# GinZhu/RDST

Measured on AMD Instinct MI355X. Metric: SR patches/sec fwd+bwd, RDST-E1 x4 64->256, higher is better.
Workload: dtype bf16; 1 GPU; RDST-E1 x4 (RDST_E1_OASIS_example_SRx4.ini), 1x64x64 LR patches -> 256x256, step = fwd + L1 + bwd + flat-bucket grad all-reduce + Adam; global_batch=32, per_gpu_batch=32, parallelism=dp1, hip_graph=True, grad_bucket_bytes=17859844

## Files before the change

### include/rdst_hip.h

```cpp
#ifndef RDST_HIP_H
#define RDST_HIP_H

#include <stddef.h>
#include <stdint.h>

#ifdef __cplusplus
extern "C" {
#endif

#define RDST_F32 0
#define RDST_BF16 1
#define RDST_F32X3 2

#define RDST_EINVAL (-10001)
#define RDST_ENOTSUP (-10002)

#define RDST_ACT_NONE 0
#define RDST_ACT_GELU 1
#define RDST_ACT_LEAKY02 2
#define RDST_ACT_LEAKY001 3

int rdst_abi_version(void);
const char* rdst_last_error(void);

// ... 81 lines not shown

#define RDST_PREPACKED ((size_t)-1)
#define RDST_PACK_LINEAR 0
#define RDST_PACK_CONV3_FWD 1
#define RDST_PACK_LINEAR_SEC3 2
#define RDST_PACK_LINEAR_X3 3
#define RDST_PACK_CONV3_FWD_X3 4
typedef struct rdst_pack_job {
  int kind;
  const float* W; const float* gamma; const float* beta; const float* bias;
  void* out;
  int N, K;
  float s;
} rdst_pack_job;
int rdst_pack_batch(const rdst_pack_job* jobs, int njobs, void* stream);
int rdst_ln_linear_fwd_packable(int K, int N, int has_ln, int has_residual, int in_act, int dtype);
size_t rdst_conv_fwd_workspace2(int Cin, int Cout, int ksize, int dtype);
int rdst_conv_fwd_packable(int Cin, int Cout, int ksize, int shuffle_r, int has_residual, int in_act, int dtype);

int rdst_reduce_batch_begin(void);
int rdst_reduce_batch_end(void* stream);
int rdst_reduce_batch_abort(void);

int rdst_nchw_to_rows(const float* nchw, void* rows, int64_t ld, int B, int C, int H, int W,
                      int dtype, void* stream);
int rdst_rows_to_nchw(const void* rows, int64_t ld, float* nchw, int B, int C, int H, int W,
                      int dtype, void* stream);

int rdst_upsample2_fwd(const void* x, int64_t ld_x, void* y, int64_t ld_y, int B, int H, int W, int C, int dtype,
                       void* stream);
int rdst_upsample2_bwd(const void* dy, int64_t ld_dy, void* dx, int64_t ld_dx, int B, int H, int W, int C, int dtype,
                       void* stream);

int rdst_adam_step(float* param, const float* grad, float* exp_avg, float* exp_avg_sq, int64_t n,
                   float lr, float beta1, float beta2, float eps, float weight_decay, int64_t step,
                   void* stream);

size_t rdst_u_scratch_bytes(void);

int rdst_u_conv(const void* X1, int64_t ld1, int C1, int up1, const void* X2, int64_t ld2, int C2, const void* Wp,
                const float* bias, const void* add, int64_t ld_add, void* Y, int64_t ld_y, int B, int Hin, int Win, int Hout,
                int Wout, int Cout, int Npad, int ksize, int stride, int transposed, int dtype, void* stream,
                const float* bn1, float* stats, int* stats_blocks);

int rdst_u_stem_fwd(const float* img, const float* W, void* Y, int64_t ld_y, int B, int Cin, int H, int Wd, int dtype,
                    void* stream);
// ... 80 lines not shown
```

### rdst_amd/_lib.py

```python
from __future__ import annotations

import ctypes as C
import os

_HERE = os.path.dirname(os.path.abspath(__file__))
LIB_PATH = os.environ.get("RDST_HIP_LIB") or os.path.join(_HERE, "librdst_hip.so")

F32, BF16, F32X3 = 0, 1, 2
EINVAL, ENOTSUP = -10001, -10002
ACT_NONE, ACT_GELU, ACT_LEAKY02, ACT_LEAKY001 = 0, 1, 2, 3

_p, _i, _l, _f, _z = C.c_void_p, C.c_int, C.c_int64, C.c_float, C.c_size_t


class LrSchedule(C.Structure):
    MAX_MILESTONES = 16
    _fields_ = [("milestones", C.c_int64 * 16), ("lr", C.c_float * 17), ("count", C.c_int32)]


STEP_STATE_BYTES = 48
SKIP_LOSS, SKIP_NONFINITE, SKIP_PEER = 1, 2, 4

SIGNATURES = {
    "rdst_abi_version": (_i, []),
# ... 14 lines not shown
    "rdst_mlp_fwd_packable": (_i, [_i, _i, _i]),
    "rdst_mlp_fwd": (_i, [_p, _l, _p, _p, _p, _p, _p, _p, _p, _l, _p, _p, _z, _l, _i, _i, _i, _p]),
    "rdst_mlp_bwd_workspace": (_z, [_l, _i, _i]),
    "rdst_mlp_bwd": (_i, [_p, _l, _p, _p, _p, _p, _p, _p, _p, _l, _p, _l, _p, _p, _p, _p, _p, _p, _p, _z, _l, _i, _i, _i,
                          _p]),
    "rdst_wattn_fwd_lse": (_i, [_p, _l, _p, _p, _l, _p, _i, _i, _i, _i, _i, _i, _i, _f, _i, _p]),
    "rdst_wattn_bwd_lse": (_i, [_p, _l, _p, _p, _l, _p, _l, _p, _p, _l, _p, _p, _z, _i, _i, _i, _i, _i, _i, _i, _f, _i, _p]),
    "rdst_swin_attn_fwd_supported": (_i, [_i, _i, _i, _i]),
    "rdst_swin_attn_fwd_workspace": (_z, [_i]),
    "rdst_swin_attn_fwd": (_i, [_p, _l, _p, _p, _p, _p, _p, _p, _p, _p, _l, _p, _l, _p, _l, _p, _p, _z, _i, _i, _i, _i, _i, _i, _i,
                                _f, _i, _p]),
    "rdst_conv_fwd_workspace": (_z, [_i, _i, _i]),
    "rdst_conv_fwd_workspace2": (_z, [_i, _i, _i, _i]),
    "rdst_conv_fwd": (_i, [_p, _l, _i, _p, _p, _p, _l, _p, _l, _p, _z, _i, _i, _i, _i, _i, _i, _f, _i, _i, _p]),
    "rdst_conv_bwd_workspace": (_z, [_i, _i, _i, _i, _i, _i]),
    "rdst_conv_bwd": (_i, [_p, _l, _i, _p, _p, _l, _p, _l, _p, _l, _p, _p, _p, _z, _i, _i, _i, _i, _i, _i,
                           _f, _i, _i, _p]),
    "rdst_pack_batch": (_i, [_p, _i, _p]),
    "rdst_ln_linear_fwd_packable": (_i, [_i, _i, _i, _i, _i, _i]),
    "rdst_conv_fwd_packable": (_i, [_i, _i, _i, _i, _i, _i, _i]),
    "rdst_reduce_batch_begin": (_i, []),
    "rdst_reduce_batch_end": (_i, [_p]),
    "rdst_reduce_batch_abort": (_i, []),
    "rdst_wattn_fwd_drop": (_i, [_p, _l, _p, _p, _i, _p, _l, _i, _i, _i, _i, _i, _i, _i, _f, _i, _f, _p, _p]),
    "rdst_wattn_bwd_drop": (_i, [_p, _l, _p, _p, _i, _p, _l, _p, _l, _p, _p, _z, _i, _i, _i, _i, _i, _i, _i, _f, _i, _f, _p, _p]),
    "rdst_wattn_drop_mask": (_i, [_p, _i, _i, _i, _i, _i, _f, _p, _p]),
    "rdst_nchw_to_rows": (_i, [_p, _p, _l, _i, _i, _i, _i, _i, _p]),
    "rdst_rows_to_nchw": (_i, [_p, _l, _p, _i, _i, _i, _i, _i, _p]),
    "rdst_upsample2_fwd": (_i, [_p, _l, _p, _l, _i, _i, _i, _i, _i, _p]),
    "rdst_upsample2_bwd": (_i, [_p, _l, _p, _l, _i, _i, _i, _i, _i, _p]),
    "rdst_adam_step": (_i, [_p, _p, _p, _p, _l, _f, _f, _f, _f, _f, _l, _p]),
    "rdst_u_scratch_bytes": (_z, []),
    "rdst_u_conv": (_i, [_p, _l, _i, _i, _p, _l, _i, _p, _p, _p, _l, _p, _l, _i, _i, _i, _i, _i, _i, _i, _i, _i, _i, _i, _p, _p, _p,
                         C.POINTER(C.c_int)]),
    "rdst_u_bn_stats_from": (_i, [_p, _i, _l, _i, _p, _p, _f, _f, _p, _p, _p, _p, _p]),
    "rdst_u_stem_fwd": (_i, [_p, _p, _p, _l, _i, _i, _i, _i, _i, _p]),
    "rdst_u_stem_dgrad": (_i, [_p, _l, _p, _p, _p, _i, _i, _i, _i, _i, _p]),
    "rdst_u_bn_stats": (_i, [_p, _l, _l, _i, _p, _p, _f, _f, _p, _p, _p, _p, _i, _p]),
    "rdst_u_bn_apply": (_i, [_p, _l, _p, _p, _l, _p, _p, _l, _i, _p, _l, _l, _i, _i, _p]),
    "rdst_u_bn_bwd": (_i, [_p, _l, _p, _l, _p, _l, _p, _p, _l, _p, _l, _p, _l, _l, _i, _p, _i, _p]),
    "rdst_u_maxpool_fwd": (_i, [_p, _l, _p, _l, _p, _i, _i, _i, _i, _i, _p]),
    "rdst_u_maxpool_bwd": (_i, [_p, _l, _p, _p, _l, _p, _l, _i, _i, _i, _i, _i, _p]),
    "rdst_u_sumpool2": (_i, [_p, _l, _p, _l, _p, _l, _i, _i, _i, _i, _i, _p]),
    "rdst_u_pair_loss_fwd": (_i, [_p, _l, _p, _l, _l, _i, _i, _f, _i, _p, _p, _i, _p]),
    "rdst_u_pair_loss_bwd": (_i, [_p, _l, _p, _l, _l, _i, _i, _f, _p, _p, _l, _p, _l, _i, _p]),
    "rdst_u_dice_fwd": (_i, [_p, _l, _p, _l, _p, _l, _i, _i, _f, _f, _i, _p, _p, _p, _i, _p]),
# ... 66 lines not shown
```

### rdst_amd/csrc/conv.h

```cpp
#pragma once
#include "common.h"

struct ConvGeom {
  int B, H, W;
  int Cin, Cout;
  int ks, pad;
  int r;
  __host__ __device__ __forceinline__ int64_t pixels() const { return (int64_t)B * H * W; }
  __device__ __forceinline__ void decode(int64_t p, int& b, int& y, int& x) const {
    const int hw = H * W;
    b = (int)(p / hw);
    const int q = (int)(p - (int64_t)b * hw);
    y = q / W;
    x = q - y * W;
  }
  __device__ __forceinline__ void out_rc(int b, int y, int x, int co, int64_t& row, int& c) const {
    if (r == 1) {
      row = ((int64_t)b * H + y) * W + x;
      c = co;
      return;
    }
    const int r2 = r * r;
    c = co / r2;
    const int rem = co - c * r2, i = rem / r, j = rem - i * r;
    row = ((int64_t)b * (H * r) + y * r + i) * (int64_t)(W * r) + x * r + j;
  }
};

template <typename T>
int conv_fwd_mfma(const T* X, int64_t ldx, int in_act, const float* Wc, const float* bias, const T* R, int64_t ldr,
                  T* Y, int64_t ldy, const ConvGeom& g, float s, bool split, hipStream_t st);
template <typename T>
const T* plain_dy(const T* dY, int64_t lddy, const ConvGeom& g, void* scratch, int64_t& ld_out, hipStream_t st, int& rc);
template <typename T>
int conv_dgrad_mfma(const T* X, int64_t ldx, int in_act, const float* Wc, const T* dYp, int64_t lddyp, T* dX,
                    int64_t lddx, const T* acc, int64_t ldacc, const ConvGeom& g, float s, bool split, hipStream_t st);
template <typename T>
int conv_wgrad_mfma(const T* X, int64_t ldx, int in_act, const T* dYp, int64_t lddyp, float* dW, float* dbias,
                    float* slab, const ConvGeom& g, float s, bool split, hipStream_t st);
size_t conv_mfma_scratch_bytes(const ConvGeom& g);

int conv_c1_fwd_bf16(const bf16* X, int64_t ldx, int in_act, const float* Wc, const float* bias, const bf16* R, int64_t ldr, bf16* Y,
                     int64_t ldy, const ConvGeom& g, float s, hipStream_t st);
int conv_c1_bwd_bf16(const bf16* X, int64_t ldx, int in_act, const float* Wc, const bf16* dY, int64_t lddy, bf16* dX,
                     int64_t lddx, const bf16* acc, int64_t ldacc, float* dW, float* dbias, float* slab, const ConvGeom& g,
                     float s, hipStream_t st);
size_t conv_c1_slab_floats(int Cin);
int conv_in1_fwd_bf16(const bf16* X, int64_t ldx, int in_act, const float* Wc, const float* bias, const bf16* R, int64_t ldr, bf16* Y,
                      int64_t ldy, const ConvGeom& g, float s, hipStream_t st);
int conv_in1_wgrad_bf16(const bf16* X, int64_t ldx, int in_act, const bf16* dY, int64_t lddy, float* dW, float* dbias, float* slab,
                        const ConvGeom& g, float s, hipStream_t st);
size_t conv_in1_slab_floats(int Cout);

size_t conv3_pack_bytes(int Cin, int Cout);
int conv3_fwd_shape(int Cin, int Cout, int ks, int r, bool has_res, int in_act);
int conv3_fwd_bf16(const bf16* X, int64_t ldx, int in_act, const float* Wc, const float* bias, const bf16* R, int64_t ldr,
                   bf16* Y, int64_t ldy, const ConvGeom& g, float s, void* wpack, bool prepacked, hipStream_t st);
int conv3_dgrad_bf16(const float* Wc, const bf16* dY, int64_t lddy, bf16* dX, int64_t lddx, const bf16* acc, int64_t ldacc,
                     int in_act, const ConvGeom& g, float s, void* wpack, hipStream_t st);
size_t conv3_wgrad_slab_bytes(int Cin, int Cout);
int conv3_wgrad_bf16(const bf16* X, int64_t ldx, int in_act, const bf16* dY, int64_t lddy, float* dW, float* dbias, float* slab,
                     const ConvGeom& g, float s, hipStream_t st);

size_t conv3x_pack_bytes(int Cin, int Cout);
int conv3x_fwd_shape(int Cin, int Cout, int ks, int r, bool has_res, int in_act);
int conv3x_fwd_f32(const float* X, int64_t ldx, int in_act, const float* Wc, const float* bias, const float* R, int64_t ldr,
                   float* Y, int64_t ldy, const ConvGeom& g, float s, void* wpack, bool prepacked, hipStream_t st);
int conv3x_dgrad_f32(const float* Wc, const float* dY, int64_t lddy, float* dX, int64_t lddx, const float* acc, int64_t ldacc,
                     int in_act, const ConvGeom& g, float s, void* wpack, hipStream_t st);
// ... 12 lines not shown
```

### rdst_amd/csrc/conv.hip

```cpp
#include "common.h"
#include "gemm_valu.h"
#include "conv.h"

namespace {

template <typename T>
struct ConvA {
  static constexpr bool kFast = true;
  const T* X; int64_t ldx; ConvGeom g; int act;
  __device__ __forceinline__ float operator()(int64_t p, int64_t k) const {
    const int tap = (int)(k / g.Cin), ci = (int)(k - (int64_t)tap * g.Cin);
    const int ky = tap / g.ks, kx = tap - ky * g.ks;
    int b, y, x;
    g.decode(p, b, y, x);
    const int yy = y + ky - g.pad, xx = x + kx - g.pad;
    if (yy < 0 || yy >= g.H || xx < 0 || xx >= g.W) return 0.f;
    return apply_act(to_f32<T>(X[(((int64_t)b * g.H + yy) * g.W + xx) * ldx + ci]), act);
  }
};
template <typename T>
struct ConvAT {
  static constexpr bool kFast = false;
  ConvA<T> a;
  __device__ __forceinline__ float operator()(int64_t p, int n) const { return a(p, n); }
};
// ... 99 lines not shown
int fwd_t(const T* X, int64_t ldx, int in_act, const float* Wc, const float* bias, const T* R, int64_t ldr, T* Y,
          int64_t ldy, const ConvGeom& g, float s, void* wpack, bool prepacked, bool split, hipStream_t st) {
  if constexpr (sizeof(T) == 2) {
    if (int rc = conv_c1_fwd_bf16(X, ldx, in_act, Wc, bias, R, ldr, Y, ldy, g, s, st); rc != RDST_ENOTSUP) return rc;
    if (int rc = conv_in1_fwd_bf16(X, ldx, in_act, Wc, bias, R, ldr, Y, ldy, g, s, st); rc != RDST_ENOTSUP) return rc;
    if (int rc = conv3_fwd_bf16(X, ldx, in_act, Wc, bias, R, ldr, Y, ldy, g, s, wpack, prepacked, st); rc != RDST_ENOTSUP) return rc;
  }
  if constexpr (sizeof(T) == 4) {
    if (int rc = conv_c1x_fwd_f32(X, ldx, in_act, Wc, bias, R, ldr, Y, ldy, g, s, st); rc != RDST_ENOTSUP) return rc;
    if (int rc = conv_in1x_fwd_f32(X, ldx, in_act, Wc, bias, R, ldr, Y, ldy, g, s, st); rc != RDST_ENOTSUP) return rc;
  }
  if constexpr (sizeof(T) == 4) {
    if (split)
      if (int rc = conv3x_fwd_f32(X, ldx, in_act, Wc, bias, R, ldr, Y, ldy, g, s, wpack, prepacked, st); rc != RDST_ENOTSUP) return rc;
  }
  if (int rc = conv_fwd_mfma<T>(X, ldx, in_act, Wc, bias, R, ldr, Y, ldy, g, s, split, st); rc != RDST_ENOTSUP) return rc;
  ConvA<T> la{X, ldx, g, in_act};
  ConvB lb{Wc, g};
  ConvFwdEp<T> ep{bias, R, ldr, Y, ldy, g, s};
  return gemm_valu_launch(la, lb, ep, g.pixels(), g.Cout, (int64_t)g.ks * g.ks * g.Cin, 1, st, "conv_fwd");
}

template <typename T>
int bwd_t(const T* X, int64_t ldx, int in_act, const float* Wc, const T* dY, int64_t lddy, T* dX, int64_t lddx,
          const T* acc, int64_t ldacc, float* dW, float* dbias, float* wsp, const ConvGeom& g, float s, bool split, hipStream_t st) {
  const int64_t wtotal = (int64_t)g.Cout * g.Cin * g.ks * g.ks;
  void* wpack = wsp;
  wsp = reinterpret_cast<float*>(reinterpret_cast<char*>(wsp) + conv3x_pack_bytes(g.Cin, g.Cout));
  float* w3slab = wsp;
  wsp = reinterpret_cast<float*>(reinterpret_cast<char*>(wsp) + (g.ks == 3 ? conv3_wgrad_slab_bytes(g.Cin, g.Cout) : 0));
  float* slab = wsp;
  float* small = slab + (int64_t)kMaxSplits * wtotal;
  char* mscr = reinterpret_cast<char*>(small + (int64_t)kSmallBlocks * g.Cout + 64);
  if constexpr (sizeof(T) == 2) {
    float* c1slab = reinterpret_cast<float*>(mscr + conv_mfma_scratch_bytes(ConvGeom{g.B, g.H, g.W, g.Cin, g.Cout, g.ks, g.pad, 2}));
    if (int rc = conv_c1_bwd_bf16(X, ldx, in_act, Wc, dY, lddy, dX, lddx, acc, ldacc, dW, dbias, c1slab, g, s, st); rc != RDST_ENOTSUP)
      return rc;
    if (!dX && (dW || dbias) && g.r == 1) {
      if (int rc = conv_in1_wgrad_bf16(X, ldx, in_act, dY, lddy, dW, dbias, c1slab, g, s, st); rc != RDST_ENOTSUP) return rc;
    }
  }
  if constexpr (sizeof(T) == 4) {
    float* c1slab = reinterpret_cast<float*>(mscr + conv_mfma_scratch_bytes(ConvGeom{g.B, g.H, g.W, g.Cin, g.Cout, g.ks, g.pad, 2}));
    if (int rc = conv_c1x_bwd_f32(X, ldx, in_act, Wc, dY, lddy, dX, lddx, acc, ldacc, dW, dbias, c1slab, g, s, st); rc != RDST_ENOTSUP)
      return rc;
    if (!dX && (dW || dbias) && g.r == 1) {
      if (int rc = conv_in1x_wgrad_f32(X, ldx, in_act, dY, lddy, dW, dbias, c1slab, g, s, st); rc != RDST_ENOTSUP) return rc;
    }
  }
  bool dxdone = false;
  if constexpr (sizeof(T) == 2) {
    if (dX) {
      const int rc = conv3_dgrad_bf16(Wc, dY, lddy, dX, lddx, acc, ldacc, in_act, g, s, wpack, st);
      if (rc == 0) dxdone = true;
      else if (rc != RDST_ENOTSUP) return rc;
    }
    if (dW || dbias) {
      const int rc = conv3_wgrad_bf16(X, ldx, in_act, dY, lddy, dW, dbias, w3slab, g, s, st);
      if (rc == 0) { dW = nullptr; dbias = nullptr; }
      else if (rc != RDST_ENOTSUP) return rc;
    }
    if ((dxdone || !dX) && !dW && !dbias) return 0;
  }
  if constexpr (sizeof(T) == 4) {
    if (dX && split) {
      const int rc = conv3x_dgrad_f32(Wc, dY, lddy, dX, lddx, acc, ldacc, in_act, g, s, wpack, st);
      if (rc == 0) dxdone = true;
      else if (rc != RDST_ENOTSUP) return rc;
    }
    if ((dW || dbias) && split) {
      const int rc = conv3x_wgrad_f32(X, ldx, in_act, dY, lddy, dW, dbias, w3slab, g, s, st);
      if (rc == 0) { dW = nullptr; dbias = nullptr; }
      else if (rc != RDST_ENOTSUP) return rc;
    }
    if ((dxdone || !dX) && !dW && !dbias) return 0;
  }
  int prc = 0;
  int64_t ldp = lddy;
  const T* dYp = plain_dy<T>(dY, lddy, g, mscr, ldp, st, prc);
  if (prc) return prc;
  float* mslab = reinterpret_cast<float*>(mscr + (g.r > 1 ? (size_t)g.pixels() * g.Cout * 4 : 0));
  bool wdone = false;
  if (dW || dbias) {
    const int rc = conv_wgrad_mfma<T>(X, ldx, in_act, dYp, ldp, dW, dbias, mslab, g, s, split, st);
    if (rc == 0) wdone = true;
    else if (rc != RDST_ENOTSUP) return rc;
  }
  if (!wdone && dbias) {
    ConvDyCol<T> f{dY, lddy, g, s};
    if (int rc = colsum_launch(f, g.pixels(), g.Cout, small, kSmallBlocks, dbias, st, "conv_dbias")) return rc;
  }
  if (!wdone && dW) {
    ConvDyAT<T> la{dY, lddy, g, s};
    ConvAT<T> lb{ConvA<T>{X, ldx, g, in_act}};
    ConvSlabEp ep{slab, g};
    const int splits = wgrad_splits(g);
    const int z = gemm_valu_splits(g.pixels(), splits);
    int rc = gemm_valu_launch(la, lb, ep, g.Cout, g.ks * g.ks * g.Cin, g.pixels(), splits, st, "conv_wgrad");
    if (!rc) rc = slab_reduce(slab, dW, z, wtotal, st);
    if (rc) return rc;
  }
  if (dX && !dxdone) {
    int rc = conv_dgrad_mfma<T>(X, ldx, in_act, Wc, dYp, ldp, dX, lddx, acc, ldacc, g, s, split, st);
    if (rc == RDST_ENOTSUP) {
      ConvDyA<T> la{dY, lddy, g, s};
      ConvBd lb{Wc, g};
      ConvDxEp<T> ep{X, ldx, dX, lddx, in_act, acc, ldacc};
      rc = gemm_valu_launch(la, lb, ep, g.pixels(), g.Cin, (int64_t)g.ks * g.ks * g.Cout, 1, st, "conv_dgrad");
    }
    if (rc) return rc;
  }
  return 0;
}

int make_geom(ConvGeom& g, int B, int H, int W, int Cin, int Cout, int ks, int r, const char* who) {
  if (B <= 0 || H <= 0 || W <= 0 || Cin <= 0 || Cout <= 0) return rdst_fail(RDST_EINVAL, "%s: non-positive dimension", who);
  if (ks != 1 && ks != 3) return rdst_fail(RDST_ENOTSUP, "%s: kernel size %d (1 or 3)", who, ks);
  if (r < 1 || Cout % (r * r)) return rdst_fail(RDST_EINVAL, "%s: Cout=%d not divisible by shuffle^2=%d", who, Cout, r * r);
  if ((int64_t)B * H * W * r * r >= (1ll << 31)) return rdst_fail(RDST_EINVAL, "%s: more than 2^31 output pixels", who);
  g.B = B; g.H = H; g.W = W; g.Cin = Cin; g.Cout = Cout; g.ks = ks; g.pad = ks / 2; g.r = r;
  return 0;
}

template <typename T>
__global__ void __launch_bounds__(256) nchw_to_rows_kernel(const float* __restrict__ src, T* __restrict__ rows, int64_t ld,
                                                           int B, int C, int64_t HW) {
  const int64_t i = (int64_t)blockIdx.x * 256 + threadIdx.x;
  if (i >= (int64_t)B * HW * C) return;
  const int c = (int)(i % C);
  const int64_t bp = i / C, b = bp / HW, p = bp - b * HW;
  rows[bp * ld + c] = from_f32<T>(src[(b * C + c) * HW + p]);
}
template <typename T>
__global__ void __launch_bounds__(256) rows_to_nchw_kernel(const T* __restrict__ rows, int64_t ld, float* __restrict__ dst,
                                                           int B, int C, int64_t HW) {
// ... 95 lines not shown
```

### rdst_amd/csrc/conv_c1.hip

```cpp
#include "common.h"
#include "gemm_valu.h"
#include "conv.h"
#include "mfma.h"

namespace {

typedef float f32x2 __attribute__((ext_vector_type(2)));

struct C1Args {
  const bf16* X; int64_t ldx;
  const float* W;
  const float* bias;
  const bf16* dY; int64_t lddy;
  bf16* Y; int64_t ldy;
  bf16* dX; int64_t lddx; const bf16* Acc; int64_t ldacc;
  float* slab;
  ConvGeom g; float s;
  int tiles_x, tiles_y; int64_t ntiles;
};

constexpr int C1_THREADS = 256;
constexpr int C1_TH = 8, C1_TW = 32, C1_HH = C1_TH + 2, C1_HW = C1_TW + 2, C1_NPIX = C1_HH * C1_HW, C1_PS = 144;

__device__ __forceinline__ void c1_unpack8(const u32x4_a4& v, float (&f)[8]) {
// ... 423 lines not shown
  hipLaunchKernelGGL(conv_c1_dgrad_kernel<true>, dim3(grid), dim3(C1_THREADS), 0, st, p);
  return rdst_launch_status("conv_in1_fwd");
}
int conv_in1_wgrad_bf16(const bf16* X, int64_t ldx, int in_act, const bf16* dY, int64_t lddy, float* dW, float* dbias, float* slab,
                        const ConvGeom& g, float s, hipStream_t st) {
  if (!in1_ok(g, in_act) || ((uintptr_t)dY & 3) || (lddy & 1)) return RDST_ENOTSUP;
  C1Args p{};
  ConvGeom gm = g;
  gm.Cin = g.Cout; gm.Cout = 1;
  p.X = dY; p.ldx = lddy; p.dY = X; p.lddy = ldx; p.g = gm; p.s = s; p.slab = slab;
  const int grid = c1_grid(p, 1024);
  hipLaunchKernelGGL(conv_c1_wgrad_kernel<true>, dim3(grid), dim3(C1_THREADS), 0, st, p);
  if (int rc = rdst_launch_status("conv_in1_wgrad")) return rc;
  const int n = g.Cout * 9, row = n + g.Cout;
  float* red = slab + (size_t)grid * row;
  if (int rc = slab_reduce(slab, red, grid, row, st)) return rc;
  if (dW) (void)hipMemcpyAsync(dW, red, sizeof(float) * n, hipMemcpyDeviceToDevice, st);
  if (dbias) (void)hipMemcpyAsync(dbias, red + n, sizeof(float) * g.Cout, hipMemcpyDeviceToDevice, st);
  return 0;
}

int conv_c1_bwd_bf16(const bf16* X, int64_t ldx, int in_act, const float* Wc, const bf16* dY, int64_t lddy, bf16* dX,
                     int64_t lddx, const bf16* acc, int64_t ldacc, float* dW, float* dbias, float* slab, const ConvGeom& g,
                     float s, hipStream_t st) {
  if (g.Cin == 1 && g.Cout == 1 && g.ks == 1 && g.r == 1 && in_act == 0 && !dW && !dbias && dX)
    return pw11_launch(dY, lddy, Wc, nullptr, acc, ldacc, dX, lddx, g.pixels(), s, st, "conv_pw11_dgrad");
  if (!c1_ok(g, in_act) || ((uintptr_t)X & 3) || (ldx & 1) || ((uintptr_t)dX & 3) || (lddx & 1) || ((uintptr_t)acc & 3) || (ldacc & 1))
    return RDST_ENOTSUP;
  C1Args p{};
  p.X = X; p.ldx = ldx; p.W = Wc; p.dY = dY; p.lddy = lddy; p.dX = dX; p.lddx = lddx; p.Acc = acc; p.ldacc = ldacc;
  p.g = g; p.s = s; p.slab = slab;
  if (dW || dbias) {
    const int grid = c1_grid(p, 1024);
    hipLaunchKernelGGL(conv_c1_wgrad_kernel<false>, dim3(grid), dim3(C1_THREADS), 0, st, p);
    if (int rc = rdst_launch_status("conv_c1_wgrad")) return rc;
    const int n = g.Cin * 9;
    float* red = slab + (size_t)grid * (n + 1);
    if (int rc = slab_reduce(slab, red, grid, n + 1, st)) return rc;
    if (dW) (void)hipMemcpyAsync(dW, red, sizeof(float) * n, hipMemcpyDeviceToDevice, st);
    if (dbias) (void)hipMemcpyAsync(dbias, red + n, sizeof(float), hipMemcpyDeviceToDevice, st);
  }
  if (dX) {
    const int grid = c1_grid(p, 1024);
    hipLaunchKernelGGL(conv_c1_dgrad_kernel<false>, dim3(grid), dim3(C1_THREADS), 0, st, p);
    if (int rc = rdst_launch_status("conv_c1_dgrad")) return rc;
  }
  return 0;
}
```

### rdst_amd/csrc/reduce_batch.h

```cpp
#pragma once
#include "common.h"

namespace rbatch {
enum SumMap {
  MAP_COPY = 0,
  MAP_LINEAR = 1,
  MAP_MLP = 2,
  MAP_DTABLE = 3,
  MAP_T = 4,
};
struct SumJob {
  const float* slab; int nwg; int64_t stride; int tot; int map;
  int g4;
  int a2, b2;
  float* out; float* out2; float* out3;
  int a, b;
  float s;
};
struct FinJob {
  const float* G; const float* Wt; const float* gamma; const float* beta;
  int N, K, Kx; float s;
  float* dW; float* dbias; float* dgamma; float* dbeta;
};
int sum(const SumJob& j, hipStream_t st);
int finish(const FinJob& j, hipStream_t st);
}
```

### rdst_amd/csrc/reduce_batch.hip

```cpp
#include "reduce_batch.h"
#include <vector>

namespace rbatch {
namespace {

constexpr int MAXJ = 16;
struct SumBatch { SumJob j[MAXJ]; int first[MAXJ + 1]; int n; };
struct FinBatch { FinJob j[MAXJ]; int first[MAXJ + 1]; int n; };

thread_local bool g_active = false;
thread_local std::vector<SumJob> g_sums;
thread_local std::vector<FinJob> g_fins;

__device__ __forceinline__ void emit(const SumJob& J, int n, int c, int i, float a) {
  if (J.map == MAP_COPY) {
    J.out[J.g4 ? n * J.b2 + c : i] = a;
  } else if (J.map == MAP_LINEAR) {
    const int K = J.a, Kx = J.b;
    if (!J.g4) { n = i / Kx; c = i - n * Kx; }
    if (c < K) { if (J.out) J.out[(int64_t)n * K + c] = a * J.s; }
    else if (c == K && J.out2) J.out2[n] = a * J.s;
  } else if (J.map == MAP_MLP) {
    const int C = J.a, hid = J.b, n1 = hid * (C + 1);
    if (i < n1) J.out[i] = a;
// ... 134 lines not shown
      blocks += (bt.j[q].K + 7) / 8;
    }
    bt.first[bt.n] = blocks;
    if (blocks == 0) continue;
    hipLaunchKernelGGL(batched_ln_finish_kernel, dim3((unsigned)blocks), dim3(1024), 0, st, bt);
    if (int rc = rdst_launch_status("batched_ln_finish")) return rc;
  }
  return 0;
}

}

int sum(const SumJob& j, hipStream_t st) {
  if (g_active) { g_sums.push_back(j); return 0; }
  return launch_sums(&j, 1, st);
}
int finish(const FinJob& j, hipStream_t st) {
  if (g_active) { g_fins.push_back(j); return 0; }
  return launch_fins(&j, 1, st);
}

}

extern "C" int rdst_reduce_batch_begin(void) {
  if (rbatch::g_active) return rdst_fail(RDST_EINVAL, "rdst_reduce_batch_begin: a batch is already open on this thread");
  rbatch::g_active = true;
  rbatch::g_sums.clear();
  rbatch::g_fins.clear();
  return 0;
}

extern "C" int rdst_reduce_batch_end(void* stream) {
  if (!rbatch::g_active) return rdst_fail(RDST_EINVAL, "rdst_reduce_batch_end: no open batch");
  rbatch::g_active = false;
  hipStream_t st = (hipStream_t)stream;
  int rc = rbatch::launch_sums(rbatch::g_sums.data(), (int)rbatch::g_sums.size(), st);
  if (!rc) rc = rbatch::launch_fins(rbatch::g_fins.data(), (int)rbatch::g_fins.size(), st);
  rbatch::g_sums.clear();
  rbatch::g_fins.clear();
  return rc;
}

extern "C" int rdst_reduce_batch_abort(void) {
  rbatch::g_active = false;
  rbatch::g_sums.clear();
  rbatch::g_fins.clear();
  return 0;
}
```

### rdst_amd/ops.py

```python
from __future__ import annotations

import os
import threading
import weakref

from typing import Optional

import torch

from . import _lib
from ._lib import ACT_GELU, ACT_LEAKY001, ACT_LEAKY02, ACT_NONE, BF16, F32, F32X3


F32_SPLIT = False
_scope_tls = threading.local()


def set_f32_split(on: bool) -> None:
    global F32_SPLIT
    F32_SPLIT = bool(on)


class compute_scope:

    def __init__(self, code: Optional[int]):
        if code not in (None, F32, _lib.F32X3, BF16):
            raise ValueError(f"rdst_amd: bad compute code {code!r}")
        self.code = code

    def __enter__(self):
        self.prev = getattr(_scope_tls, "code", None)
        if self.code is not None:
            _scope_tls.code = self.code
# ... 441 lines not shown
class _ReduceBatchState(threading.local):

    EPOCH = 0

    def __init__(self):
        self.depth, self.keep, self.fresh = 0, [], 0
        self.owner, self.mixed = -1, False
        self.epoch = type(self).EPOCH

    @staticmethod
    def _task():
        return torch._C._current_graph_task_id()

    def _foreign(self):
        if self.depth > 0 and self._task() != self.owner:
            self.mixed = True
        return self.mixed

    def _drop_stale(self, lib):
        if self.epoch != type(self).EPOCH:
            self.abandon(lib)
            self.epoch = type(self).EPOCH

    def _flush(self, lib):
        try:
            _lib.check(lib.rdst_reduce_batch_end(_stream()), "rdst_reduce_batch_end")
        finally:
            self.keep = []
            self.fresh = 0

    def begin(self, lib):
        self._drop_stale(lib)
        if self.depth == 0:
            _lib.check(lib.rdst_reduce_batch_begin(), "rdst_reduce_batch_begin")
            self.owner = self._task()
            self.mixed = False
        self.depth += 1

    def begin_layer(self, lib):
        self._drop_stale(lib)
        if self.depth > 0:
            if self.owner == self._task():
                self.abandon(lib)
            else:
                self.mixed = True
        self.begin(lib)

    def end(self, lib, keep=None):
        if keep:
            self.keep.extend(keep)
        self.depth -= 1
        if self.depth == 0:
            self._flush(lib)

    def settle(self, lib):
        self._drop_stale(lib)
        if self.depth > 0 and (self.fresh or self._foreign()):
            self._flush(lib)
            _lib.check(lib.rdst_reduce_batch_begin(), "rdst_reduce_batch_begin")
        elif self.depth == 0:
            self.fresh = 0

    def abandon(self, lib):
        if self.depth > 0:
            _lib.check(lib.rdst_reduce_batch_abort(), "rdst_reduce_batch_abort")
        self.depth = 0
        self.keep = []
        self.fresh = 0
        self.mixed = False


_ReduceBatch = _ReduceBatchState()


def reset_backward_state() -> None:
    type(_ReduceBatch).EPOCH += 1
    if _lib.loaded():
        _ReduceBatch._drop_stale(_lib.load())


class GradSink:

    def __init__(self):
        self.extra = None
        self.batch_open = False

    def take(self):
        e, self.extra = self.extra, None
        return e

    def take_batch(self):
        b, self.batch_open = self.batch_open, False
        return b


class _DenseJoin(torch.autograd.Function):

    @staticmethod
    def forward(ctx, prefix, new, buf, sink=None):
        ctx.c = prefix.shape[-1]
        ctx.sink = sink
# ... 249 lines not shown
            _wsp, wptr, nws = _packed_workspace([(PACK_CONV3_FWD_X3 if code == F32X3 else PACK_CONV3_FWD, w, None, None, None, Cout,
                                                  Cin, out_scale, nb)], nb, x.device)
        _lib.check(lib.rdst_conv_fwd(x_r.data_ptr(), ldx, int(in_act), w.data_ptr(), _ptr(b), _ptr(r_r), ldr,
                                     y.data_ptr(), ldy, wptr, nws, B, H, W, Cin, Cout, k, float(out_scale), r,
                                     code, _stream()), "rdst_conv_fwd")
        ctx.bias_ref = b
        ctx.save_for_backward(x_r, w)
        ctx.meta = (B, H, W, Cin, Cout, k, ldx, int(in_act), float(out_scale), r, residual is not None, code)
        return y

    @staticmethod
    def backward(ctx, dy):
        x, w = ctx.saved_tensors
        B, H, W, Cin, Cout, k, ldx, in_act, out_scale, r, has_res, code = ctx.meta
        lib = _lib.load()
        dy_r, lddy = _rows(dy)
        need = ctx.needs_input_grad
        dev = x.device
        dx = torch.empty((B, H, W, Cin), dtype=x.dtype, device=dev) if need[0] else None
        dw = _grad_like(w) if need[1] else None
        db = _bias_grad(ctx, need[2])
        nbytes = lib.rdst_conv_bwd_workspace(B, H, W, Cin, Cout, k)
        wsp = _workspace(nbytes, dev)
        _lib.check(lib.rdst_conv_bwd(x.data_ptr(), ldx, in_act, w.data_ptr(), dy_r.data_ptr(), lddy, _ptr(dx), Cin,
                                     None, 0, _ptr(dw), _ptr(db), wsp.data_ptr(), nbytes, B, H, W, Cin, Cout, k,
                                     out_scale, r, code, _stream()), "rdst_conv_bwd")
        _ReduceBatch.settle(lib)
        dres = dy if (has_res and need[3]) else None
        return dx, dw, db, dres, None, None, None, None


def conv_rows(x: torch.Tensor, weight: torch.Tensor, bias: Optional[torch.Tensor], *, in_act: int = ACT_NONE,
              residual: Optional[torch.Tensor] = None, out_scale: float = 1.0, shuffle: int = 1, out_slot=None) -> torch.Tensor:
    return _ConvRows.apply(x, weight, bias, residual, in_act, out_scale, shuffle, out_slot)


class _NchwToRows(torch.autograd.Function):
    @staticmethod
    def forward(ctx, x, dtype):
        _need_gpu(x)
        lib = _lib.load()
        B, C, H, W = x.shape
        xs = x.detach().float().contiguous()
        rows = torch.empty((B, H, W, C), dtype=dtype, device=x.device)
        _lib.check(lib.rdst_nchw_to_rows(xs.data_ptr(), rows.data_ptr(), C, B, C, H, W, _elt_code(rows), _stream()),
                   "rdst_nchw_to_rows")
        return rows

    @staticmethod
# ... 57 lines not shown
```

### rdst_amd/trainer.py

```python
from __future__ import annotations

import math
import time
from typing import Callable, Dict, Optional, Sequence

import torch
import torch.distributed as dist
import torch.nn.functional as F

from . import dp
from .optim import FlatAdam

GUARD_OFF = 1e8


class DPTrainStep:

    RECORD_FLUSH = 4096

    def __init__(self, net: torch.nn.Module, lr: float = 1e-4, betas=(0.9, 0.99), eps: float = 1e-8,
                 weight_decay: float = 0.0, milestones: Optional[Sequence[int]] = None, gamma: float = 0.5,
                 loss_threshold: float = GUARD_OFF, loss_fn: Optional[Callable] = None, group=None,
                 graph: bool = False, graph_warmup: int = 2, device_guard: bool = False,
                 max_grad_norm: Optional[float] = None, skip_nonfinite: bool = False):
        self.device_guard = bool(device_guard)
        self.max_grad_norm = None if max_grad_norm is None else float(max_grad_norm)
        self.skip_nonfinite = bool(skip_nonfinite)
        if self.device_guard and not all(p.is_cuda for p in net.parameters()):
            raise ValueError("DPTrainStep(device_guard=True): the guard is a HIP kernel, the network must be on a GPU")
        if not self.device_guard and (self.max_grad_norm is not None or self.skip_nonfinite):
            raise ValueError("DPTrainStep: max_grad_norm and skip_nonfinite need device_guard=True")
        self.net = net
        self.group = group
# ... 72 lines not shown
                out.append(x)
        return out

    def _flush_records(self) -> None:
        for n, vals in self._pending.items():
            if not vals:
                continue
            keeps = self._pending_keep.get(n) or [None] * len(vals)
            self.training_loss_records.setdefault(n, []).extend(self._filter_records(vals, keeps))
        self._pending = {}
        self._pending_keep = {}

    def loss_records(self) -> Dict[str, list]:
        self._flush_records()
        return self.training_loss_records

    def fwd_bwd(self, inputs: torch.Tensor, targets: torch.Tensor) -> torch.Tensor:
        self.bucket.detach_grads()
        out = self.net(inputs)
        loss = self._loss(out, targets)
        if self._loss_buf is None:
            self._loss_buf = torch.zeros((), dtype=torch.float32, device=inputs.device)
        self._loss_buf.copy_(loss.detach())
        loss.backward()
        self.bucket.gather()
        return self._loss_buf

    def capture(self, inputs: torch.Tensor, targets: torch.Tensor) -> bool:
        import contextlib
        self._static = (inputs.detach().clone(), targets.detach().clone())
        torch.cuda.synchronize()
        g = torch.cuda.CUDAGraph()
        try:
            with (self.capture_hook() if self.capture_hook is not None else contextlib.nullcontext()):
                with torch.cuda.graph(g):
                    self.fwd_bwd(*self._static)
                    if self._update_in_graph():
                        self._finish_step()
        except Exception as e:
            import warnings
            warnings.warn(f"rdst_amd.trainer: HIP-graph capture failed ({type(e).__name__}: {e}); running eagerly")
            torch.cuda.synchronize()
            from . import ops
            ops.reset_backward_state()
            dp._OFFERED = {}
            self.bucket.gather()
            self.use_graph, self.graph, self._static, self._graph_report = False, None, None, None
# ... 166 lines not shown
```

Before: 1898 patches/s.

## Overlap conv weight-grad and batched reductions on a side stream during backward

Adds a per-device side stream with event-based fork/join. During backward, conv weight-gradient kernels (c1 and 3x3 wgrad) and the batched reduction launches run on that stream, concurrently with the data-gradient work on the main stream. Python-side bookkeeping keeps the input tensors alive until a join, and the trainer enables the side path only around loss.backward(). The aim is to fill idle GPU capacity with independent wgrad work. The cost is more synchronisation complexity, extra events in the captured graph, and possible contention between the two streams.

```diff
diff --git a/include/rdst_hip.h b/include/rdst_hip.h
--- a/include/rdst_hip.h
+++ b/include/rdst_hip.h
@@ -127,6 +127,10 @@
 int rdst_reduce_batch_end(void* stream);
 int rdst_reduce_batch_abort(void);
 
+int rdst_side_enable(int on);
+int rdst_side_join(void* stream);
+int rdst_side_reset(void);
+
 int rdst_nchw_to_rows(const float* nchw, void* rows, int64_t ld, int B, int C, int H, int W,
                       int dtype, void* stream);
 int rdst_rows_to_nchw(const void* rows, int64_t ld, float* nchw, int B, int C, int H, int W,
diff --git a/rdst_amd/_lib.py b/rdst_amd/_lib.py
--- a/rdst_amd/_lib.py
+++ b/rdst_amd/_lib.py
@@ -60,6 +60,9 @@
     "rdst_reduce_batch_begin": (_i, []),
     "rdst_reduce_batch_end": (_i, [_p]),
     "rdst_reduce_batch_abort": (_i, []),
+    "rdst_side_enable": (_i, [_i]),
+    "rdst_side_join": (_i, [_p]),
+    "rdst_side_reset": (_i, []),
     "rdst_wattn_fwd_drop": (_i, [_p, _l, _p, _p, _i, _p, _l, _i, _i, _i, _i, _i, _i, _i, _f, _i, _f, _p, _p]),
     "rdst_wattn_bwd_drop": (_i, [_p, _l, _p, _p, _i, _p, _l, _p, _l, _p, _p, _z, _i, _i, _i, _i, _i, _i, _i, _f, _i, _f, _p, _p]),
     "rdst_wattn_drop_mask": (_i, [_p, _i, _i, _i, _i, _i, _f, _p, _p]),
diff --git a/rdst_amd/csrc/conv.h b/rdst_amd/csrc/conv.h
--- a/rdst_amd/csrc/conv.h
+++ b/rdst_amd/csrc/conv.h
@@ -44,7 +44,7 @@
                      int64_t ldy, const ConvGeom& g, float s, hipStream_t st);
 int conv_c1_bwd_bf16(const bf16* X, int64_t ldx, int in_act, const float* Wc, const bf16* dY, int64_t lddy, bf16* dX,
                      int64_t lddx, const bf16* acc, int64_t ldacc, float* dW, float* dbias, float* slab, const ConvGeom& g,
-                     float s, hipStream_t st);
+                     float s, hipStream_t st, hipStream_t wst);
 size_t conv_c1_slab_floats(int Cin);
 int conv_in1_fwd_bf16(const bf16* X, int64_t ldx, int in_act, const float* Wc, const float* bias, const bf16* R, int64_t ldr, bf16* Y,
                       int64_t ldy, const ConvGeom& g, float s, hipStream_t st);
diff --git a/rdst_amd/csrc/conv.hip b/rdst_amd/csrc/conv.hip
--- a/rdst_amd/csrc/conv.hip
+++ b/rdst_amd/csrc/conv.hip
@@ -1,6 +1,7 @@
 #include "common.h"
 #include "gemm_valu.h"
 #include "conv.h"
+#include "reduce_batch.h"
 
 namespace {
 
@@ -146,8 +147,9 @@
 }
 
 template <typename T>
-int bwd_t(const T* X, int64_t ldx, int in_act, const float* Wc, const T* dY, int64_t lddy, T* dX, int64_t lddx,
-          const T* acc, int64_t ldacc, float* dW, float* dbias, float* wsp, const ConvGeom& g, float s, bool split, hipStream_t st) {
+int bwd_impl(const T* X, int64_t ldx, int in_act, const float* Wc, const T* dY, int64_t lddy, T* dX, int64_t lddx,
+             const T* acc, int64_t ldacc, float* dW, float* dbias, float* wsp, const ConvGeom& g, float s, bool split, hipStream_t st,
+             hipStream_t wst) {
   const int64_t wtotal = (int64_t)g.Cout * g.Cin * g.ks * g.ks;
   void* wpack = wsp;
   wsp = reinterpret_cast<float*>(reinterpret_cast<char*>(wsp) + conv3x_pack_bytes(g.Cin, g.Cout));
@@ -158,7 +160,7 @@
   char* mscr = reinterpret_cast<char*>(small + (int64_t)kSmallBlocks * g.Cout + 64);
   if constexpr (sizeof(T) == 2) {
     float* c1slab = reinterpret_cast<float*>(mscr + conv_mfma_scratch_bytes(ConvGeom{g.B, g.H, g.W, g.Cin, g.Cout, g.ks, g.pad, 2}));
-    if (int rc = conv_c1_bwd_bf16(X, ldx, in_act, Wc, dY, lddy, dX, lddx, acc, ldacc, dW, dbias, c1slab, g, s, st); rc != RDST_ENOTSUP)
+    if (int rc = conv_c1_bwd_bf16(X, ldx, in_act, Wc, dY, lddy, dX, lddx, acc, ldacc, dW, dbias, c1slab, g, s, st, wst); rc != RDST_ENOTSUP)
       return rc;
     if (!dX && (dW || dbias) && g.r == 1) {
       if (int rc = conv_in1_wgrad_bf16(X, ldx, in_act, dY, lddy, dW, dbias, c1slab, g, s, st); rc != RDST_ENOTSUP) return rc;
@@ -180,7 +182,7 @@
       else if (rc != RDST_ENOTSUP) return rc;
     }
     if (dW || dbias) {
-      const int rc = conv3_wgrad_bf16(X, ldx, in_act, dY, lddy, dW, dbias, w3slab, g, s, st);
+      const int rc = conv3_wgrad_bf16(X, ldx, in_act, dY, lddy, dW, dbias, w3slab, g, s, wst);
       if (rc == 0) { dW = nullptr; dbias = nullptr; }
       else if (rc != RDST_ENOTSUP) return rc;
     }
@@ -193,7 +195,7 @@
       else if (rc != RDST_ENOTSUP) return rc;
     }
     if ((dW || dbias) && split) {
-      const int rc = conv3x_wgrad_f32(X, ldx, in_act, dY, lddy, dW, dbias, w3slab, g, s, st);
+      const int rc = conv3x_wgrad_f32(X, ldx, in_act, dY, lddy, dW, dbias, w3slab, g, s, wst);
       if (rc == 0) { dW = nullptr; dbias = nullptr; }
       else if (rc != RDST_ENOTSUP) return rc;
     }
@@ -235,6 +237,18 @@
     if (rc) return rc;
   }
   return 0;
+}
+
+template <typename T>
+int bwd_t(const T* X, int64_t ldx, int in_act, const float* Wc, const T* dY, int64_t lddy, T* dX, int64_t lddx,
+          const T* acc, int64_t ldacc, float* dW, float* dbias, float* wsp, const ConvGeom& g, float s, bool split, hipStream_t st) {
+  rside::Fork f;
+  f.run = st;
+  if (dX && (dW || dbias))
+    if (int rc = rside::fork_begin(st, f)) return rc;
+  int rc = bwd_impl<T>(X, ldx, in_act, Wc, dY, lddy, dX, lddx, acc, ldacc, dW, dbias, wsp, g, s, split, st, f.run);
+  const int rc2 = rside::fork_end(f);
+  return rc ? rc : rc2;
 }
 
 int make_geom(ConvGeom& g, int B, int H, int W, int Cin, int Cout, int ks, int r, const char* who) {
diff --git a/rdst_amd/csrc/conv_c1.hip b/rdst_amd/csrc/conv_c1.hip
--- a/rdst_amd/csrc/conv_c1.hip
+++ b/rdst_amd/csrc/conv_c1.hip
@@ -469,7 +469,7 @@
 
 int conv_c1_bwd_bf16(const bf16* X, int64_t ldx, int in_act, const float* Wc, const bf16* dY, int64_t lddy, bf16* dX,
                      int64_t lddx, const bf16* acc, int64_t ldacc, float* dW, float* dbias, float* slab, const ConvGeom& g,
-                     float s, hipStream_t st) {
+                     float s, hipStream_t st, hipStream_t wst) {
   if (g.Cin == 1 && g.Cout == 1 && g.ks == 1 && g.r == 1 && in_act == 0 && !dW && !dbias && dX)
     return pw11_launch(dY, lddy, Wc, nullptr, acc, ldacc, dX, lddx, g.pixels(), s, st, "conv_pw11_dgrad");
   if (!c1_ok(g, in_act) || ((uintptr_t)X & 3) || (ldx & 1) || ((uintptr_t)dX & 3) || (lddx & 1) || ((uintptr_t)acc & 3) || (ldacc & 1))
@@ -479,13 +479,13 @@
   p.g = g; p.s = s; p.slab = slab;
   if (dW || dbias) {
     const int grid = c1_grid(p, 1024);
-    hipLaunchKernelGGL(conv_c1_wgrad_kernel<false>, dim3(grid), dim3(C1_THREADS), 0, st, p);
+    hipLaunchKernelGGL(conv_c1_wgrad_kernel<false>, dim3(grid), dim3(C1_THREADS), 0, wst, p);
     if (int rc = rdst_launch_status("conv_c1_wgrad")) return rc;
     const int n = g.Cin * 9;
     float* red = slab + (size_t)grid * (n + 1);
-    if (int rc = slab_reduce(slab, red, grid, n + 1, st)) return rc;
-    if (dW) (void)hipMemcpyAsync(dW, red, sizeof(float) * n, hipMemcpyDeviceToDevice, st);
-    if (dbias) (void)hipMemcpyAsync(dbias, red + n, sizeof(float), hipMemcpyDeviceToDevice, st);
+    if (int rc = slab_reduce(slab, red, grid, n + 1, wst)) return rc;
+    if (dW) (void)hipMemcpyAsync(dW, red, sizeof(float) * n, hipMemcpyDeviceToDevice, wst);
+    if (dbias) (void)hipMemcpyAsync(dbias, red + n, sizeof(float), hipMemcpyDeviceToDevice, wst);
   }
   if (dX) {
     const int grid = c1_grid(p, 1024);
diff --git a/rdst_amd/csrc/reduce_batch.h b/rdst_amd/csrc/reduce_batch.h
--- a/rdst_amd/csrc/reduce_batch.h
+++ b/rdst_amd/csrc/reduce_batch.h
@@ -25,3 +25,10 @@
 int sum(const SumJob& j, hipStream_t st);
 int finish(const FinJob& j, hipStream_t st);
 }
+
+namespace rside {
+constexpr int SIDE_REDUCE = 1, SIDE_CONV = 2;
+struct Fork { hipStream_t run = nullptr; void* dev = nullptr; unsigned long long cap = 0; };
+int fork_begin(hipStream_t st, Fork& f);
+int fork_end(Fork& f);
+}
diff --git a/rdst_amd/csrc/reduce_batch.hip b/rdst_amd/csrc/reduce_batch.hip
--- a/rdst_amd/csrc/reduce_batch.hip
+++ b/rdst_amd/csrc/reduce_batch.hip
@@ -1,4 +1,6 @@
 #include "reduce_batch.h"
+#include <atomic>
+#include <mutex>
 #include <vector>
 
 namespace rbatch {
@@ -180,6 +182,144 @@
 
 }
 
+namespace rside {
+
+constexpr int MAXDEV = 16;
+constexpr int RING = 4;
+constexpr unsigned long long NO_CAPTURE = 0;
+
+struct Dev {
+  hipStream_t side = nullptr;
+  hipEvent_t ev[RING] = {};
+  bool ready = false;
+  int next = 0;
+  int pending = -1;
+  unsigned long long pending_cap = NO_CAPTURE;
+};
+
+std::atomic<int> g_enabled{0};
+std::mutex g_mu;
+Dev g_dev[MAXDEV];
+
+int hip_fail(hipError_t e, const char* what) { return rdst_fail(-(int)e, "%s: %s", what, hipGetErrorString(e)); }
+
+int where(hipStream_t st, int& dev, unsigned long long& cap) {
+  hipError_t e = st ? hipStreamGetDevice(st, &dev) : hipGetDevice(&dev);
+  if (e != hipSuccess) return hip_fail(e, "rdst_side: device of the stream");
+  hipStreamCaptureStatus cs = hipStreamCaptureStatusNone;
+  unsigned long long id = 0;
+  e = hipStreamGetCaptureInfo(st, &cs, &id);
+  if (e != hipSuccess) return hip_fail(e, "rdst_side: hipStreamGetCaptureInfo");
+  if (cs == hipStreamCaptureStatusInvalidated) return rdst_fail(RDST_EINVAL, "rdst_side: the stream's capture is invalidated");
+  cap = cs == hipStreamCaptureStatusActive ? id + 1 : NO_CAPTURE;
+  return 0;
+}
+
+int create(Dev& d, int dev) {
+  int cur = -1;
+  hipError_t e = hipGetDevice(&cur);
+  if (e == hipSuccess && cur != dev) e = hipSetDevice(dev);
+  if (e == hipSuccess) e = hipStreamCreateWithFlags(&d.side, hipStreamNonBlocking);
+  for (int k = 0; k < RING && e == hipSuccess; ++k) e = hipEventCreateWithFlags(&d.ev[k], hipEventDisableTiming);
+  if (cur >= 0 && cur != dev) (void)hipSetDevice(cur);
+  if (e != hipSuccess) {
+    for (int k = 0; k < RING; ++k)
+      if (d.ev[k]) { (void)hipEventDestroy(d.ev[k]); d.ev[k] = nullptr; }
+    if (d.side) { (void)hipStreamDestroy(d.side); d.side = nullptr; }
+    return hip_fail(e, "rdst_side: creating the side stream");
+  }
+  d.ready = true;
+  d.next = 0;
+  d.pending = -1;
+  return 0;
+}
+
+int wait_pending(Dev& d, hipStream_t st, unsigned long long cap, const char* who) {
+  if (d.pending < 0) return 0;
+  if (d.pending_cap == cap) {
+    hipError_t e = hipStreamWaitEvent(st, d.ev[d.pending], 0);
+    if (e != hipSuccess) return hip_fail(e, who);
+  } else if (d.pending_cap == NO_CAPTURE) {
+    return rdst_fail(RDST_EINVAL, "%s: side work issued before this stream capture began is still pending (rdst_side_join first)", who);
+  }
+  d.pending = -1;
+  return 0;
+}
+
+int open_generation(hipStream_t st, Dev*& d, unsigned long long& cap, bool reductions = true) {
+  int dev = 0;
+  if (int rc = where(st, dev, cap)) return rc;
+  if (dev < 0 || dev >= MAXDEV) return 0;
+  Dev& D = g_dev[dev];
+  if (!D.ready) {
+    if (cap != NO_CAPTURE) return 0;
+    if (int rc = create(D, dev)) return rc;
+  }
+  if (reductions) {
+    if (int rc = wait_pending(D, st, cap, "rdst_reduce_batch_end")) return rc;
+  } else if (D.pending >= 0 && D.pending_cap != cap) {
+    if (D.pending_cap == NO_CAPTURE) return rdst_fail(RDST_EINVAL, "rdst_side: side work issued before this stream capture began is still pending");
+    D.pending = -1;
+  }
+  hipError_t e = hipEventRecord(D.ev[D.next], st);
+  if (e == hipSuccess) e = hipStreamWaitEvent(D.side, D.ev[D.next], 0);
+  if (e != hipSuccess) return hip_fail(e, "rdst_reduce_batch_end: forking the side stream");
+  d = &D;
+  return 0;
+}
+
+int wait_only(hipStream_t st) {
+  int dev = 0;
+  unsigned long long cap = 0;
+  if (int rc = where(st, dev, cap)) return rc;
+  if (dev < 0 || dev >= MAXDEV || !g_dev[dev].ready) return 0;
+  return wait_pending(g_dev[dev], st, cap, "rdst_reduce_batch_end");
+}
+
+int close_generation(Dev& d, unsigned long long cap) {
+  const int slot = d.next + 1;
+  hipError_t e = hipEventRecord(d.ev[slot], d.side);
+  if (e != hipSuccess) return hip_fail(e, "rdst_reduce_batch_end: closing the side generation");
+  d.pending = slot;
+  d.pending_cap = cap;
+  d.next = (d.next + 2) % RING;
+  return 0;
+}
+
+int forget_all(const char* who) {
+  std::lock_guard<std::mutex> lk(g_mu);
+  int rc = 0;
+  for (Dev& d : g_dev) {
+    if (!d.ready || d.pending < 0) continue;
+    if (d.pending_cap == NO_CAPTURE) {
+      hipError_t e = hipStreamSynchronize(d.side);
+      if (e != hipSuccess && !rc) rc = hip_fail(e, who);
+    }
+    d.pending = -1;
+  }
+  return rc;
+}
+
+int fork_begin(hipStream_t st, Fork& f) {
+  f.run = st;
+  f.dev = nullptr;
+  if (!(g_enabled.load(std::memory_order_relaxed) & SIDE_CONV)) return 0;
+  std::lock_guard<std::mutex> lk(g_mu);
+  Dev* d = nullptr;
+  if (int rc = open_generation(st, d, f.cap, false)) return rc;
+  if (d) { f.dev = d; f.run = d->side; }
+  return 0;
+}
+int fork_end(Fork& f) {
+  if (!f.dev) return 0;
+  std::lock_guard<std::mutex> lk(g_mu);
+  Dev* d = static_cast<Dev*>(f.dev);
+  f.dev = nullptr;
+  return close_generation(*d, f.cap);
+}
+
+}
+
 extern "C" int rdst_reduce_batch_begin(void) {
   if (rbatch::g_active) return rdst_fail(RDST_EINVAL, "rdst_reduce_batch_begin: a batch is already open on this thread");
   rbatch::g_active = true;
@@ -192,8 +332,23 @@
   if (!rbatch::g_active) return rdst_fail(RDST_EINVAL, "rdst_reduce_batch_end: no open batch");
   rbatch::g_active = false;
   hipStream_t st = (hipStream_t)stream;
-  int rc = rbatch::launch_sums(rbatch::g_sums.data(), (int)rbatch::g_sums.size(), st);
-  if (!rc) rc = rbatch::launch_fins(rbatch::g_fins.data(), (int)rbatch::g_fins.size(), st);
+  int rc = 0;
+  if (const int bits = rside::g_enabled.load(std::memory_order_relaxed)) {
+    std::lock_guard<std::mutex> lk(rside::g_mu);
+    rside::Dev* d = nullptr;
+    unsigned long long cap = 0;
+    rc = (bits & rside::SIDE_REDUCE) ? rside::open_generation(st, d, cap) : rside::wait_only(st);
+    hipStream_t run = d ? d->side : st;
+    if (!rc) rc = rbatch::launch_sums(rbatch::g_sums.data(), (int)rbatch::g_sums.size(), run);
+    if (!rc) rc = rbatch::launch_fins(rbatch::g_fins.data(), (int)rbatch::g_fins.size(), run);
+    if (d) {
+      const int rc2 = rside::close_generation(*d, cap);
+      if (!rc) rc = rc2;
+    }
+  } else {
+    rc = rbatch::launch_sums(rbatch::g_sums.data(), (int)rbatch::g_sums.size(), st);
+    if (!rc) rc = rbatch::launch_fins(rbatch::g_fins.data(), (int)rbatch::g_fins.size(), st);
+  }
   rbatch::g_sums.clear();
   rbatch::g_fins.clear();
   return rc;
@@ -203,5 +358,19 @@
   rbatch::g_active = false;
   rbatch::g_sums.clear();
   rbatch::g_fins.clear();
-  return 0;
-}
+  return rside::forget_all("rdst_reduce_batch_abort");
+}
+
+extern "C" int rdst_side_enable(int on) { return rside::g_enabled.exchange(on & (rside::SIDE_REDUCE | rside::SIDE_CONV)); }
+
+extern "C" int rdst_side_join(void* stream) {
+  std::lock_guard<std::mutex> lk(rside::g_mu);
+  hipStream_t st = (hipStream_t)stream;
+  int dev = 0;
+  unsigned long long cap = 0;
+  if (int rc = rside::where(st, dev, cap)) return rc;
+  if (dev < 0 || dev >= rside::MAXDEV || !rside::g_dev[dev].ready) return 0;
+  return rside::wait_pending(rside::g_dev[dev], st, cap, "rdst_side_join");
+}
+
+extern "C" int rdst_side_reset(void) { return rside::forget_all("rdst_side_reset"); }
diff --git a/rdst_amd/ops.py b/rdst_amd/ops.py
--- a/rdst_amd/ops.py
+++ b/rdst_amd/ops.py
@@ -8,7 +8,7 @@
 
 import torch
 
-from . import _lib
+from . import _lib, side
 from ._lib import ACT_GELU, ACT_LEAKY001, ACT_LEAKY02, ACT_NONE, BF16, F32, F32X3
 
 
@@ -496,12 +496,20 @@
             self.abandon(lib)
             self.epoch = type(self).EPOCH
 
-    def _flush(self, lib):
+    def _flush(self, lib, join=False):
+        on_side = side.enabled()
         try:
             _lib.check(lib.rdst_reduce_batch_end(_stream()), "rdst_reduce_batch_end")
         finally:
+            if on_side:
+                side.park(self.keep)
             self.keep = []
             self.fresh = 0
+        if on_side:
+            from . import dp
+            side.release_older()
+            if join or not dp._OFFERED:
+                side.join()
 
     def begin(self, lib):
         self._drop_stale(lib)
@@ -530,7 +538,7 @@
     def settle(self, lib):
         self._drop_stale(lib)
         if self.depth > 0 and (self.fresh or self._foreign()):
-            self._flush(lib)
+            self._flush(lib, join=True)
             _lib.check(lib.rdst_reduce_batch_begin(), "rdst_reduce_batch_begin")
         elif self.depth == 0:
             self.fresh = 0
@@ -551,6 +559,7 @@
     type(_ReduceBatch).EPOCH += 1
     if _lib.loaded():
         _ReduceBatch._drop_stale(_lib.load())
+    side.reset()
 
 
 class GradSink:
@@ -846,9 +855,16 @@
         db = _bias_grad(ctx, need[2])
         nbytes = lib.rdst_conv_bwd_workspace(B, H, W, Cin, Cout, k)
         wsp = _workspace(nbytes, dev)
+        forked = side.conv_enabled() and dx is not None and (dw is not None or db is not None)
+        fresh = _ReduceBatch.fresh
         _lib.check(lib.rdst_conv_bwd(x.data_ptr(), ldx, in_act, w.data_ptr(), dy_r.data_ptr(), lddy, _ptr(dx), Cin,
                                      None, 0, _ptr(dw), _ptr(db), wsp.data_ptr(), nbytes, B, H, W, Cin, Cout, k,
                                      out_scale, r, code, _stream()), "rdst_conv_bwd")
+        if forked:
+            from . import dp
+            side.park_current([x, dy_r, wsp])
+            if fresh or not dp._OFFERED:
+                side.join()
         _ReduceBatch.settle(lib)
         dres = dy if (has_res and need[3]) else None
         return dx, dw, db, dres, None, None, None, None
diff --git a/rdst_amd/side.py b/rdst_amd/side.py
--- /dev/null
+++ b/rdst_amd/side.py
@@ -0,0 +1,88 @@
+from __future__ import annotations
+
+import os
+import threading
+
+import torch
+
+from . import _lib
+
+SIDE_BRANCH = os.environ.get("RDST_SIDE_BRANCH", "1") != "0"
+SIDE_CONV = os.environ.get("RDST_SIDE_CONV", "1") != "0"
+
+_lock = threading.Lock()
+_on = False
+_handle = None
+_parked: dict = {}
+
+
+def _stream() -> int:
+    return torch.cuda.current_stream().cuda_stream
+
+
+def enabled() -> bool:
+    return _on
+
+
+def conv_enabled() -> bool:
+    return _on and SIDE_CONV
+
+
+def enable() -> bool:
+    global _on, _handle
+    bits = (1 if SIDE_BRANCH else 0) | (2 if SIDE_CONV else 0)
+    if not bits:
+        return False
+    if _handle is None:
+        _handle = _lib.load()
+    _handle.rdst_side_enable(bits)
+    _on = True
+    return True
+
+
+def disable() -> bool:
+    global _on
+    was = _on
+    if _handle is not None:
+        was = bool(_handle.rdst_side_enable(0)) or was
+    _on = False
+    return was
+
+
+def park(tensors) -> None:
+    with _lock:
+        _parked.setdefault(torch.cuda.current_device(), []).append(list(tensors))
+
+
+def park_current(tensors) -> None:
+    with _lock:
+        gens = _parked.setdefault(torch.cuda.current_device(), [])
+        if not gens:
+            gens.append([])
+        gens[-1].extend(t for t in tensors if t is not None)
+
+
+def release_older() -> None:
+    with _lock:
+        gens = _parked.get(torch.cuda.current_device())
+        if gens and len(gens) > 1:
+            del gens[:-1]
+
+
+def join() -> None:
+    if _handle is None:
+        return
+    try:
+        _lib.check(_handle.rdst_side_join(_stream()), "rdst_side_join")
+    finally:
+        with _lock:
+            _parked.pop(torch.cuda.current_device(), None)
+
+
+def reset() -> None:
+    if _handle is not None:
+        try:
+            _lib.check(_handle.rdst_side_reset(), "rdst_side_reset")
+        finally:
+            with _lock:
+                _parked.clear()
diff --git a/rdst_amd/trainer.py b/rdst_amd/trainer.py
--- a/rdst_amd/trainer.py
+++ b/rdst_amd/trainer.py
@@ -8,7 +8,7 @@
 import torch.distributed as dist
 import torch.nn.functional as F
 
-from . import dp
+from . import dp, side
 from .optim import FlatAdam
 
 GUARD_OFF = 1e8
@@ -127,7 +127,14 @@
         if self._loss_buf is None:
             self._loss_buf = torch.zeros((), dtype=torch.float32, device=inputs.device)
         self._loss_buf.copy_(loss.detach())
-        loss.backward()
+        side.enable()
+        try:
+            loss.backward()
+        finally:
+            try:
+                side.join()
+            finally:
+                side.disable()
         self.bucket.gather()
         return self._loss_buf
 
```

Measured after the change: 1936 patches/s, median of 6. 2.0% higher.
